# EdanToledo/Stoix

Hardware: AMD Instinct MI355X
Metric: env steps/sec (whole node), Anakin PPO on Brax Ant at 1/2/4/8 MI355X (higher is better)
Workload: dtype bf16; 1 GPU; model=ppo_mlp_256x2_tanh_normal, global_batch=4096, seq_len=128, parallelism=dp1, env=brax/ant, epochs=4, num_minibatches=16

## Files before the change

stoix_amd/ops/csrc/bind.cpp:

```cpp
#include <torch/extension.h>
#include <ATen/hip/HIPContext.h>

#include <cstdint>

extern "C" {
void launch_cartpole_step(float*, const long*, int*, float*, int*, float*,
                          int*, float*, float*, float*, float*, unsigned char*,
                          unsigned char*, int, int, uint64_t, unsigned int*,
                          unsigned int, int, void*);
void launch_ant_step(float*, const float*, int*, float*, int*, float*, int*,
                     float*, float*, float*, float*, unsigned char*,
                     unsigned char*, int, int, uint64_t, unsigned int*,
                     unsigned int, int, void*);
void launch_humanoid_step(float*, const float*, int*, float*, int*, float*,
                          int*, float*, float*, float*, float*,
                          unsigned char*, unsigned char*, int, int, uint64_t,
                          unsigned int*, unsigned int, int, void*);
void launch_ant_reset(float*, int, uint64_t, uint32_t, void*);
void launch_gae(const float*, const float*, const float*, const float*,
                const unsigned char*, float*, float*, int, int, float, void*);
void launch_lambda_returns(const float*, const float*, const float*, float*,
                           int, int, float, void*);
void launch_vtrace(const float*, const float*, const float*, const float*,
                   const float*, float*, float*, int, int, float, float,
// ... 30 lines not shown
                             float, float, float, uint64_t, uint64_t,
                             unsigned int*, unsigned int*, unsigned int,
                             void*);
void launch_linear_silu(const void*, const void*, const float*, void*,
                        void*, int, int, int, int, void*);
void launch_silu_fwd(const void*, void*, long, void*);
void launch_silu_bwd(const void*, const void*, void*, long, void*);
void launch_silu_heads_fwd(const void*, const void*, const void*, const void*,
                           const void*, void*, void*, void*, int, int, void*);
void launch_heads_bwd_silu(const void*, const void*, const void*, const void*,
                           const void*, void*, int, int, void*);
void launch_ppo_gather(const long*, int, const float*, int, int,
                       const float*, int,
                       const float*, const float*, const float*, const float*,
                       void*, float*, float*, float*, float*, float*,
                       const float*, const float*, void*);
void launch_ppo_head_loss(const void*, const void*, const float*,
                          const float*, const float*, const float*,
                          const float*, void*, void*, void*, float*, int,
                          int, float, float, float, float, float, float,
                          float, uint64_t, unsigned int*, unsigned int, int,
                          void*);
void launch_wgrad(const void*, const void*, float*, long, long, long, int,
                  int, int, int, int, int, void*);
void launch_slab_reduce(float*, void*, long, long, float*, long*, void*);
void launch_bump_add(unsigned int*, unsigned int, void*);
void launch_tr16_probe(const void*, float*, int, void*);
int launch_wgrad_pair(const void*, const void*, float*, long, long, long, int,
                      const void*, const void*, float*, long, long, long, int,
                      int, int, int, int, void*);
void launch_slab_reduce_pair(const float*, void*, long, long, float*, long*,
                             const float*, void*, long, long, float*, long*,
                             void*);
void launch_sumtree_update(float*, const long*, const float*, long, int, int,
                           void*);
void launch_sumtree_sample(const float*, const float*, long*, long, int, int,
                           int, void*);
void launch_policy_value_step_disc(const float*, const void*, const float*,
                                   const void*, const float*, const void*,
                                   const float*, const void*, const float*,
                                   const void*, const float*, const void*,
                                   const float*, float*, long*, float*,
                                   float*, const float*, const float*, int,
                                   int, int, int, int, uint64_t,
                                   unsigned int*, unsigned int, int, void*);
void launch_ppo_head_loss_disc(const void*, const void*, const long*,
                               const float*, const float*, const float*,
                               const float*, void*, void*, void*, float*,
                               int, int, float, float, float, void*);
void launch_ppo_gather_disc(const long*, int, const float*, int, int,
                            const long*, const float*, const float*,
                            const float*, const float*, void*, long*, float*,
                            float*, float*, float*, const float*,
                            const float*, void*);
void launch_rnn_scan(const float*, const void*, const float*,
                     const unsigned char*, const float*, const float*,
                     float*, float*, float*, int, int, int, int, void*);
void launch_rnn_scan_train_fwd(const float*, const void*, const float*,
                               const unsigned char*, const float*,
                               const float*, float*, float*, float*, float*,
                               float*, int, int, int, int, void*);
void launch_rnn_scan_bwd(const float*, const float*, const float*,
                         const float*, const float*, const float*,
                         const float*, const float*, const unsigned char*,
                         const void*, float*, float*, float*, float*, int,
                         int, int, int, void*);
// ... 420 lines not shown
  launch_rollout_step_ant(
      obs_io.data_ptr<float>(), env_state.data_ptr<float>(),
      step_count.data_ptr<int>(), ep_return.data_ptr<float>(),
      ep_length.data_ptr<int>(), last_ep_return.data_ptr<float>(),
      last_ep_length.data_ptr<int>(), W1a.data_ptr(), b1a.data_ptr<float>(),
      W2a.data_ptr(), b2a.data_ptr<float>(), Wha.data_ptr(),
      bha.data_ptr<float>(), W1c.data_ptr(), b1c.data_ptr<float>(),
      W2c.data_ptr(), b2c.data_ptr<float>(), Wvc.data_ptr(),
      bvc.data_ptr<float>(), buf_obs.data_ptr<float>(),
      buf_action.data_ptr<float>(), buf_logp.data_ptr<float>(),
      buf_value.data_ptr<float>(), buf_bootstrap.data_ptr<float>(),
      buf_reward.data_ptr<float>(), buf_discount.data_ptr<float>(),
      buf_steptype.data_ptr<unsigned char>(), B, OBS, ACT, HID,
      (int)max_episode_steps, (float)min_scale, (float)aff_scale,
      (float)aff_shift, (float)log_aff_scale, (uint64_t)policy_seed,
      (uint64_t)env_seed, (unsigned int*)policy_draw.data_ptr<int>(),
      (unsigned int*)env_draw.data_ptr<int>(), (unsigned int)draw_offset,
      cur_stream());
}

void linear_silu(torch::Tensor X, torch::Tensor W, torch::Tensor bias,
                 torch::Tensor Z, torch::Tensor H, int64_t do_silu) {
  CHK(X, torch::kBFloat16);
  CHK(W, torch::kBFloat16);
  CHK(bias, torch::kFloat32);
  int S = X.size(0), K = X.size(1), N = W.size(0);
  TORCH_CHECK(S % 128 == 0 && N % 128 == 0 && K % 32 == 0,
              "linear_silu tile constraints");
  void* h = H.numel() > 0 ? H.data_ptr() : nullptr;
  launch_linear_silu(X.data_ptr(), W.data_ptr(), bias.data_ptr<float>(),
                     Z.data_ptr(), h, S, K, N, (int)do_silu, cur_stream());
}

void silu_fwd(torch::Tensor z, torch::Tensor h) {
  CHK(z, torch::kBFloat16);
  TORCH_CHECK(z.numel() % 8 == 0, "silu_fwd needs numel % 8 == 0");
  launch_silu_fwd(z.data_ptr(), h.data_ptr(), z.numel(), cur_stream());
}

void silu_bwd(torch::Tensor dh, torch::Tensor z, torch::Tensor dz) {
  CHK(z, torch::kBFloat16);
  TORCH_CHECK(z.numel() % 8 == 0, "silu_bwd needs numel % 8 == 0");
  launch_silu_bwd(dh.data_ptr(), z.data_ptr(), dz.data_ptr(), z.numel(),
                  cur_stream());
}

int check_stacked_heads(const torch::Tensor& Z2, const torch::Tensor& other,
                        const torch::Tensor& Wh, const torch::Tensor& Wv,
                        const torch::Tensor& rows16, const torch::Tensor& rows1,
                        bool rows1_optional, int* hid) {
  CHK(Z2, torch::kBFloat16);
  CHK(other, torch::kBFloat16);
  CHK(rows16, torch::kBFloat16);
  CHK(rows1, torch::kBFloat16);
  TORCH_CHECK(Z2.dim() == 3 && Z2.size(0) == 2,
              "fused heads need stacked [2, S, HID] buffers");
  const int64_t S = Z2.size(1), HID = Z2.size(2);
  TORCH_CHECK(HID == 512 || HID == 256 || HID == 128,
              "fused heads support HID 128/256/512, got ", HID);
  TORCH_CHECK(S % 16 == 0, "fused heads need S % 16 == 0, got ", S);
  TORCH_CHECK(other.sizes() == Z2.sizes(),
              "fused heads: [2, S, HID] buffers differ in shape");
  check_fused_weight(Wh, "Wh", 16, HID);
  check_fused_weight(Wv.view({-1, 1}), "Wv", HID, 1);
  TORCH_CHECK(rows16.numel() == S * 16, "fused heads: expected [S, 16]");
  TORCH_CHECK(rows1.numel() == S || (rows1_optional && rows1.numel() == 0),
// ... 141 lines not shown
  wgrad_pair_slab_check(slab1, dW_off1, db_off1, n_valid1, K);
  return launch_wgrad_pair(
             dZ0.data_ptr(), X0.data_ptr(), slab0.data_ptr<float>(),
             (long)dW_off0, (long)db_off0, (long)slab0.size(1), (int)n_valid0,
             dZ1.data_ptr(), X1.data_ptr(), slab1.data_ptr<float>(),
             (long)dW_off1, (long)db_off1, (long)slab1.size(1), (int)n_valid1,
             (int)S, (int)N_STRIDE, (int)K, (int)variant, cur_stream()) != 0;
}

void slab_reduce_pair(torch::Tensor slab0, torch::Tensor grad0,
                      torch::Tensor sqnorm0, torch::Tensor step0,
                      torch::Tensor slab1, torch::Tensor grad1,
                      torch::Tensor sqnorm1, torch::Tensor step1) {
  CHK(slab0, torch::kFloat32);
  CHK(grad0, torch::kBFloat16);
  CHK(slab1, torch::kFloat32);
  CHK(grad1, torch::kBFloat16);
  TORCH_CHECK(slab0.dim() == 2 && slab0.size(0) == 64 && slab1.dim() == 2 &&
                  slab1.size(0) == 64, "slab_reduce_pair: slabs must be [64, n]");
  TORCH_CHECK(grad0.numel() <= slab0.size(1) && grad1.numel() <= slab1.size(1),
              "slab_reduce_pair: grad longer than a slab image");
  TORCH_CHECK((sqnorm0.numel() > 0) == (step0.numel() > 0) &&
                  (sqnorm1.numel() > 0) == (step1.numel() > 0),
              "slab_reduce_pair: sqnorm and step_t go together");
  float* sq0 = sqnorm0.numel() > 0 ? sqnorm0.data_ptr<float>() : nullptr;
  long* st0 = step0.numel() > 0 ? step0.data_ptr<long>() : nullptr;
  float* sq1 = sqnorm1.numel() > 0 ? sqnorm1.data_ptr<float>() : nullptr;
  long* st1 = step1.numel() > 0 ? step1.data_ptr<long>() : nullptr;
  launch_slab_reduce_pair(slab0.data_ptr<float>(), grad0.data_ptr(),
                          slab0.size(1), grad0.numel(), sq0, st0,
                          slab1.data_ptr<float>(), grad1.data_ptr(),
                          slab1.size(1), grad1.numel(), sq1, st1,
                          cur_stream());
}

void bump_add(torch::Tensor draw_buf, int64_t n) {
  launch_bump_add((unsigned int*)draw_buf.data_ptr<int>(), (unsigned int)n,
                  cur_stream());
}

void tr16_probe(torch::Tensor in, torch::Tensor out, int64_t base_mode) {
  CHK(in, torch::kBFloat16);
  launch_tr16_probe(in.data_ptr(), out.data_ptr<float>(), (int)base_mode,
                    cur_stream());
}

int check_c51_logits(const torch::Tensor& logits, const char* name,
                     int64_t B, int64_t A) {
  TORCH_CHECK(logits.is_cuda() && logits.is_contiguous(), name,
              " must be a contiguous GPU tensor");
  TORCH_CHECK(logits.scalar_type() == torch::kFloat32 ||
                  logits.scalar_type() == torch::kBFloat16,
              name, " must be fp32 or bf16");
  TORCH_CHECK(logits.dim() == 3 && logits.size(0) == B && logits.size(1) == A,
              name, " must be [", B, ", ", A, ", atoms]");
  TORCH_CHECK(A >= 1 && A <= 64, "c51 loss supports 1 <= A <= 64, got ", A);
  TORCH_CHECK(logits.size(2) >= 1 && logits.size(2) <= 1024,
              "c51 loss supports 1 <= atoms <= 1024, got ", logits.size(2));
  return logits.scalar_type() == torch::kBFloat16 ? 1 : 0;
}

void check_c51_vector(const torch::Tensor& t, const char* name,
                      torch::ScalarType ty, int64_t B) {
  TORCH_CHECK(t.is_cuda() && t.scalar_type() == ty && t.dim() == 1 &&
                  t.size(0) == B && t.stride(0) >= 0,
              name, " must be a GPU vector of ", B, " ", ty, " values");
// ... 389 lines not shown
        "fused clip + Adam, bf16 grads + bf16 param mirror");
  m.def("polyak", &polyak, "polyak target update");
  m.def("mfma_probe", &mfma_probe, "MFMA 16x16x32 bf16 layout probe");
  m.def("policy_value_step", &policy_value_step,
        "fused actor+critic fwd + tanh-normal sample (MFMA)");
  m.def("value_forward", &value_forward, "fused critic fwd (MFMA)");
  m.def("rollout_step_ant", &rollout_step_ant,
        "fused rollout step: policy + Ant physics + bootstrap, one launch");
  m.def("linear_silu", &linear_silu,
        "fused Linear(+bias)+SiLU forward, MFMA tiled");
  m.def("silu_fwd", &silu_fwd, "bf16 silu forward");
  m.def("silu_bwd", &silu_bwd, "bf16 silu backward");
  m.def("silu_heads_fwd", &silu_heads_fwd,
        "stacked silu forward fused with the actor/critic head GEMMs");
  m.def("heads_bwd_silu", &heads_bwd_silu,
        "head dgrads (K=16 / K=1) fused with the stacked silu backward");
  m.def("ppo_gather", &ppo_gather, "fused minibatch gather");
  m.def("ppo_head_loss", &ppo_head_loss,
        "fused PPO head fwd + losses + analytic head bwd");
  m.def("wgrad", &wgrad, "split-K MFMA weight grad + bias colsum -> slab",
        py::arg("dZ"), py::arg("X"), py::arg("slab"), py::arg("dW_off"),
        py::arg("db_off"), py::arg("n_valid"), py::arg("kpg") = 0,
        py::arg("ntb") = 0);
  m.def("slab_reduce", &slab_reduce,
        "sum wgrad slabs into flat bf16 grads (+ fused Adam prologue)");
  m.def("wgrad_pair", &wgrad_pair,
        "both nets' split-K wgrads in one pipelined launch -> slabs",
        py::arg("dZ0"), py::arg("X0"), py::arg("slab0"), py::arg("dW_off0"),
        py::arg("db_off0"), py::arg("n_valid0"), py::arg("dZ1"),
        py::arg("X1"), py::arg("slab1"), py::arg("dW_off1"),
        py::arg("db_off1"), py::arg("n_valid1"), py::arg("variant") = -1);
  m.def("slab_reduce_pair", &slab_reduce_pair,
        "both chains' slabs -> flat bf16 grads, slabs left un-zeroed");
  m.def("bump_add", &bump_add, "add N to a device RNG draw counter");
  m.def("tr16_probe", &tr16_probe, "ds_read_tr16_b64 semantics probe");
}
```

stoix_amd/ops/csrc/mlp.hip:

```cpp
#include "common.h"
#include "ant_core.h"
#include <hip/hip_bf16.h>
#include <stdexcept>
#include <string>
#include <type_traits>

typedef __bf16 bf16_t;
typedef __bf16 bf16x8 __attribute__((ext_vector_type(8)));
typedef __bf16 bf16x4 __attribute__((ext_vector_type(4)));
typedef float f32x4 __attribute__((ext_vector_type(4)));

#define MFMA_BF16_16x16x32 __builtin_amdgcn_mfma_f32_16x16x32_bf16

DEV_INLINE float bf2f(bf16_t x) { return (float)x; }
DEV_INLINE bf16_t f2bf(float x) { return (bf16_t)x; }

DEV_INLINE float silu_f(float x) {
  float s = 1.0f / (1.0f + __expf(-x));
  return x * s;
}
DEV_INLINE float silu_grad_f(float x) {
  float s = 1.0f / (1.0f + __expf(-x));
  return s * (1.0f + x * (1.0f - s));
}
// ... 587 lines not shown
    int n = n_blk + wn + nj * 16 + col_l;
    float bv = bias[n];
#pragma unroll
    for (int mi = 0; mi < 4; ++mi) {
#pragma unroll
      for (int r = 0; r < 4; ++r) {
        int m = m0 + wm + mi * 16 + g * 4 + r;
        float z = acc[mi][nj][r] + bv;
        Z[(long)m * N + n] = f2bf(z);
        if (SILU && H) H[(long)m * N + n] = f2bf(silu_f(z));
      }
    }
  }
}

extern "C" void launch_linear_silu(const void* X, const void* W,
                                   const float* bias, void* Z, void* H,
                                   int S, int K, int N, int do_silu,
                                   void* stream) {
  dim3 grid(S / LSF_BM, N / 128), block(256);
  if (do_silu) {
    hipLaunchKernelGGL(linear_silu_kernel<true>, grid, block, 0,
                       (hipStream_t)stream, (const bf16_t*)X,
                       (const bf16_t*)W, bias, (bf16_t*)Z, (bf16_t*)H, S, K,
                       N);
  } else {
    hipLaunchKernelGGL(linear_silu_kernel<false>, grid, block, 0,
                       (hipStream_t)stream, (const bf16_t*)X,
                       (const bf16_t*)W, bias, (bf16_t*)Z, (bf16_t*)H, S, K,
                       N);
  }
}


extern "C" __global__ void silu_fwd_kernel(const bf16_t* __restrict__ z,
                                           bf16_t* __restrict__ h, long n) {
  long i = ((long)blockIdx.x * blockDim.x + threadIdx.x) * 8;
  long stride = (long)gridDim.x * blockDim.x * 8;
  for (; i < n; i += stride) {
    bf16x8 zv = *reinterpret_cast<const bf16x8*>(z + i);
    bf16x8 hv;
#pragma unroll
    for (int j = 0; j < 8; ++j) hv[j] = f2bf(silu_f(bf2f(zv[j])));
    *reinterpret_cast<bf16x8*>(h + i) = hv;
  }
}

extern "C" __global__ void silu_bwd_kernel(const bf16_t* __restrict__ dh,
                                           const bf16_t* __restrict__ z,
                                           bf16_t* __restrict__ dz, long n) {
  long i = ((long)blockIdx.x * blockDim.x + threadIdx.x) * 8;
  long stride = (long)gridDim.x * blockDim.x * 8;
  for (; i < n; i += stride) {
    bf16x8 dv = *reinterpret_cast<const bf16x8*>(dh + i);
    bf16x8 zv = *reinterpret_cast<const bf16x8*>(z + i);
    bf16x8 o;
#pragma unroll
    for (int j = 0; j < 8; ++j)
      o[j] = f2bf(bf2f(dv[j]) * silu_grad_f(bf2f(zv[j])));
    *reinterpret_cast<bf16x8*>(dz + i) = o;
  }
}


DEV_INLINE void wave_lds_sync() {
  __builtin_amdgcn_fence(__ATOMIC_ACQ_REL, "wavefront");
// ... 768 lines not shown
```

stoix_amd/ops/csrc/optim.hip:

```cpp
#include "common.h"

extern "C" __global__ void grad_sqnorm_kernel(
    const float* __restrict__ grad, float* __restrict__ out, long n) {
  long tid = (long)blockIdx.x * blockDim.x + threadIdx.x;
  long stride = (long)gridDim.x * blockDim.x;
  float acc = 0.0f;
  long nvec = n / 4;
  const float4* g4 = reinterpret_cast<const float4*>(grad);
  for (long v = tid; v < nvec; v += stride) {
    float4 g = g4[v];
    acc += g.x * g.x + g.y * g.y + g.z * g.z + g.w * g.w;
  }
  for (long j = nvec * 4 + tid; j < n; j += stride) acc += grad[j] * grad[j];
#pragma unroll
  for (int off = 32; off > 0; off >>= 1) acc += __shfl_down(acc, off);
  __shared__ float warp_sums[16];
  int lane = threadIdx.x & 63;
  int wid = threadIdx.x >> 6;
  if (lane == 0) warp_sums[wid] = acc;
  __syncthreads();
  if (threadIdx.x == 0) {
    float s = 0.0f;
    int nw = (blockDim.x + 63) / 64;
    for (int w = 0; w < nw; ++w) s += warp_sums[w];
// ... 126 lines not shown
}

extern "C" void launch_fused_adam_bf16(float* param, const void* grad,
                                       float* exp_avg, float* exp_avg_sq,
                                       float* sqnorm, long* step_t,
                                       void* param_bf16, long n, float lr,
                                       float beta1, float beta2, float eps,
                                       float max_norm, float grad_scale,
                                       int do_prologue, long sqnorm_len,
                                       void* stream) {
  hipStream_t s = (hipStream_t)stream;
  if (do_prologue)
    hipLaunchKernelGGL(adam_prologue_kernel, dim3(1), dim3(1), 0, s, sqnorm,
                       step_t);
  int threads = 256;
  long want = (n / 8 + threads - 1) / threads;
  int blocks = (int)(want < 2048 ? (want > 0 ? want : 1) : 2048);
  int n_partials = 0;
  if (max_norm > 0.0f) {
    bool ordered = sqnorm_len >= 1 + (long)blocks;
    if (ordered) n_partials = blocks;
    hipLaunchKernelGGL(grad_sqnorm_bf16_kernel, dim3(blocks), dim3(threads),
                       0, s, (const opt_bf16*)grad, sqnorm,
                       ordered ? sqnorm + 1 : (float*)nullptr, n);
  }
  long want2 = (n + threads - 1) / threads;
  int blocks2 = (int)(want2 < 2048 ? (want2 > 0 ? want2 : 1) : 2048);
  hipLaunchKernelGGL(adam_update_bf16_kernel, dim3(blocks2), dim3(threads), 0,
                     s, param, (const opt_bf16*)grad, exp_avg, exp_avg_sq,
                     sqnorm, step_t, (opt_bf16*)param_bf16, n, lr, beta1,
                     beta2, eps, max_norm, grad_scale, n_partials);
}

extern "C" __global__ void polyak_kernel(const float* __restrict__ online,
                                         float* __restrict__ target,
                                         long n, float tau) {
  long i = (long)blockIdx.x * blockDim.x + threadIdx.x;
  long stride = (long)gridDim.x * blockDim.x;
  for (; i < n; i += stride)
    target[i] = tau * online[i] + (1.0f - tau) * target[i];
}

extern "C" void launch_fused_adam(float* param, const float* grad,
                                  float* exp_avg, float* exp_avg_sq,
                                  float* sqnorm, long* step_t, long n,
                                  float lr, float beta1, float beta2,
                                  float eps, float max_norm, void* stream) {
  hipStream_t s = (hipStream_t)stream;
  hipLaunchKernelGGL(adam_prologue_kernel, dim3(1), dim3(1), 0, s, sqnorm, step_t);
  int threads = 256;
  long want = (n / 4 + threads - 1) / threads;
  int blocks = (int)(want < 2048 ? (want > 0 ? want : 1) : 2048);
  if (max_norm > 0.0f) {
    hipLaunchKernelGGL(grad_sqnorm_kernel, dim3(blocks), dim3(threads), 0, s,
                       grad, sqnorm, n);
  }
  long want2 = (n + threads - 1) / threads;
  int blocks2 = (int)(want2 < 2048 ? (want2 > 0 ? want2 : 1) : 2048);
  hipLaunchKernelGGL(adam_update_kernel, dim3(blocks2), dim3(threads), 0, s,
                     param, grad, exp_avg, exp_avg_sq, sqnorm, step_t, n, lr,
                     beta1, beta2, eps, max_norm);
}

extern "C" void launch_polyak(const float* online, float* target, long n,
                              float tau, void* stream) {
  int threads = 256;
// ... 6 lines not shown
```

stoix_amd/ops/csrc/wgrad.hip:

```cpp
#include "common.h"
#include <cstdlib>
#include <hip/hip_bf16.h>

typedef __bf16 bf16_t;
typedef __bf16 bf16x8 __attribute__((ext_vector_type(8)));
typedef __bf16 bf16x4 __attribute__((ext_vector_type(4)));
typedef float f32x4 __attribute__((ext_vector_type(4)));

#define MFMA_BF16_16x16x32 __builtin_amdgcn_mfma_f32_16x16x32_bf16

#define WG_SLICES 64
#define SPAD 8

struct WgradLds {
  bf16_t dZt[4][4 * 16][32 + SPAD];
  bf16_t Xt[4][8 * 16][32 + SPAD];
};

template <int KPG, int NTB>
__launch_bounds__(256, 2) __global__ void wgrad_kernel(
    const bf16_t* __restrict__ dZ,
    const bf16_t* __restrict__ X,
    float* __restrict__ slab,
    long dW_off,
// ... 297 lines not shown
      d += __shfl_xor(d, 32);
      if (g == 0 && nb + col < N_VALID) out[db_off + nb + col] = d;
    }
  }
}

extern "C" __launch_bounds__(256) __global__ void slab_reduce_pair_kernel(
    const float* __restrict__ slab0, __bf16* __restrict__ grad0, long stride0,
    long n0, float* __restrict__ sqnorm0, long* __restrict__ step0,
    const float* __restrict__ slab1, __bf16* __restrict__ grad1, long stride1,
    long n1, float* __restrict__ sqnorm1, long* __restrict__ step1) {
  const bool second = blockIdx.y != 0;
  const float* __restrict__ slab = second ? slab1 : slab0;
  __bf16* __restrict__ grad16 = second ? grad1 : grad0;
  const long slab_stride = second ? stride1 : stride0;
  const long n = second ? n1 : n0;
  float* sqnorm = second ? sqnorm1 : sqnorm0;
  long* step_t = second ? step1 : step0;
  if (sqnorm && blockIdx.x == 0 && threadIdx.x == 0) {
    *sqnorm = 0.0f;
    *step_t += 1;
  }
  long i = (long)blockIdx.x * blockDim.x + threadIdx.x;
  long stride = (long)gridDim.x * blockDim.x;
  for (; i < n; i += stride) {
    float v[WG_SLICES];
#pragma unroll
    for (int z = 0; z < WG_SLICES; ++z) v[z] = slab[(long)z * slab_stride + i];
    float s = 0.0f;
#pragma unroll
    for (int z = 0; z < WG_SLICES; ++z) s += v[z];
    grad16[i] = (__bf16)s;
  }
}

extern "C" __global__ void tr16_probe_kernel(const bf16_t* __restrict__ in,
                                             float* __restrict__ out,
                                             int base_mode) {
  __shared__ bf16_t l[1024];
  int t = threadIdx.x;
  for (int i = t; i < 1024; i += 64) l[i] = in[i];
  __syncthreads();
  if (t >= 64) return;
  int off = 0;
  if (base_mode == 1) off = (t >> 4) * 64;
  else if (base_mode == 2) off = (t >> 4) * 128;
  bf16x4 v = __builtin_amdgcn_ds_read_tr16_b64_v4bf16(
      (__attribute__((address_space(3))) bf16x4*)&l[off]);
#pragma unroll
  for (int j = 0; j < 4; ++j) out[t * 4 + j] = (float)v[j];
}


extern "C" void launch_wgrad(const void* dZ, const void* X, float* slab,
                             long dW_off, long db_off, long slab_stride,
                             int S, int N_STRIDE, int K, int N_VALID,
                             int kpg_override, int ntb_override,
                             void* stream) {
  hipStream_t s = (hipStream_t)stream;
  int NT = (N_VALID + 15) / 16;
  int NTB = (NT % 4 == 0) ? 4 : 1;
  int KPG = 1;
  if (ntb_override > 0) NTB = ntb_override;
  if (kpg_override > 0) {
    KPG = kpg_override;
  } else if (NT <= 1) {
// ... 128 lines not shown
```

stoix_amd/systems/ppo/fused.py:

```python
from __future__ import annotations

import math
from typing import Dict, List, Optional, Tuple

import torch
import torch.nn as nn
import torch.nn.functional as F

from stoix_amd.networks.heads import NormalAffineTanhDistributionHead, ScalarCriticHead
from stoix_amd.networks.torso import MLPTorso

Tensor = torch.Tensor


def _mlp_linears(torso: nn.Module) -> Optional[List[nn.Linear]]:
    if not isinstance(torso, MLPTorso):
        return None
    lins = [m for m in torso.net if isinstance(m, nn.Linear)]
    acts = [m for m in torso.net if isinstance(m, nn.SiLU)]
    if len(lins) != 2 or len(acts) != 2 or len(list(torso.net)) != 4:
        return None
    return lins


class _Chain:

    def __init__(
        self,
        specs: List[Tuple[str, Tuple[int, ...]]],
        device,
        lr: float,
        flat16: Optional[Tensor] = None,
        grad16: Optional[Tensor] = None,
    ):
        self.lr = lr
        sizes = [int(torch.prod(torch.tensor(s)).item()) for _, s in specs]
        total = sum(sizes)
        self.flat = torch.zeros(total, dtype=torch.float32, device=device)
        self.flat16 = (
            flat16 if flat16 is not None
            else torch.zeros(total, dtype=torch.bfloat16, device=device)
        )
        self.grad16 = (
            grad16 if grad16 is not None
            else torch.zeros(total, dtype=torch.bfloat16, device=device)
        )
        self.m = torch.zeros(total, dtype=torch.float32, device=device)
        self.v = torch.zeros(total, dtype=torch.float32, device=device)
        self.sqnorm = torch.zeros(1 + 2048, dtype=torch.float32, device=device)
        self.step_t = torch.zeros(1, dtype=torch.int64, device=device)
        self.views: Dict[str, Tensor] = {}
        self.views16: Dict[str, Tensor] = {}
        self.gviews16: Dict[str, Tensor] = {}
        self.offsets: Dict[str, int] = {}
        off = 0
        for (name, shape), n in zip(specs, sizes):
            self.views[name] = self.flat[off : off + n].view(*shape)
            self.views16[name] = self.flat16[off : off + n].view(*shape)
            self.gviews16[name] = self.grad16[off : off + n].view(*shape)
            self.offsets[name] = off
            off += n
        self.numel = total
        self.slab = torch.zeros(64, total, dtype=torch.float32, device=device)

    def sync_mirror(self) -> None:
        self.flat16.copy_(self.flat)


class FusedPPOEngine:

    @staticmethod
    def try_build(learner) -> Optional["FusedPPOEngine"]:
        if learner.device.type != "cuda":
            return None
        if type(learner).policy_loss is not _base_policy_loss_func(learner):
            return None
        actor, critic = learner.actor, learner.critic
        if actor.input_layer is not None or critic.input_layer is not None:
            return None
        a_lins = _mlp_linears(actor.torso)
        c_lins = _mlp_linears(critic.torso)
        if a_lins is None or c_lins is None:
# ... 149 lines not shown
                ws.val = z(S, dtype=torch.float32)
                ws.adv = z(S, dtype=torch.float32)
                ws.tgt = z(S, dtype=torch.float32)

        self.ws = [_Ws(), _Ws()]
        self.Xmb = self.ws[0].Xmb
        self.act_mb = self.ws[0].act
        self.logp_mb = self.ws[0].logp
        self.val_mb = self.ws[0].val
        self.adv_mb = self.ws[0].adv
        self.tgt_mb = self.ws[0].tgt
        self.gather_stream = torch.cuda.Stream(dev)
        self.ev_ready = [torch.cuda.Event(), torch.cuda.Event()]
        self.ev_consumed = [torch.cuda.Event(), torch.cuda.Event()]
        self.Z1, self.H1 = z(2, S, H), z(2, S, H)
        self.Z2, self.H2 = z(2, S, H), z(2, S, H)
        self.dH2 = z(2, S, H)
        self.dZ2 = z(2, S, H)
        self.dH1 = z(2, S, H)
        self.dZ1 = z(2, S, H)
        self.heads = z(S, 16)
        self.vpred = z(S, 1)
        self.dhead = z(S, 16)
        self.dv = z(S, 1)
        self.dv16 = z(S, 16)

        import os as _os

        self.use_bmm = _os.environ.get("STOIX_FUSED_BMM", "1") != "0"
        _heads = _os.environ.get("STOIX_FUSED_HEADS", "1")
        self.fused_heads = _heads != "0"
        self.fused_vpred = _heads == "2"
        self.fused_wgrad = _os.environ.get("STOIX_FUSED_WGRAD", "1") != "0"
        self.no_vpred = z(0)
        self.prefetch = _os.environ.get("STOIX_FUSED_PREFETCH", "0") == "1"

        import torch.distributed as dist

        self.world = dist.get_world_size() if dist.is_initialized() else 1

        self.norm = bool(getattr(learner, "normalize_obs", False))
        if self.norm:
            st = learner.obs_stats
            self.nmean = st.mean
            self.nvar = (st.std ** 2).clone()
            self.gmean = st.mean.clone()
            self.gvar = self.nvar.clone()

        learner.env._hb["obs"].copy_(learner.cur_obs)


    def _adopt_params(self, a_lins, c_lins, head, critic_head) -> None:
        ac, cc = self.actor_chain, self.critic_chain
        ACT, H = self.ACT, self.H
        OBS = self.OBS
        with torch.no_grad():
            ac.views["W1"].zero_()
            cc.views["W1"].zero_()
            ac.views["W1"][:, :OBS].copy_(a_lins[0].weight)
            ac.views["b1"].copy_(a_lins[0].bias)
            ac.views["W2"].copy_(a_lins[1].weight)
            ac.views["b2"].copy_(a_lins[1].bias)
            ac.views["Wh"].zero_()
            ac.views["bh"].zero_()
            if self.discrete:
                ac.views["Wh"][0:ACT].copy_(head.linear.weight)
                ac.views["bh"][0:ACT].copy_(head.linear.bias)
            else:
                ac.views["Wh"][0:ACT].copy_(head.loc.weight)
                ac.views["Wh"][8 : 8 + ACT].copy_(head.scale.weight)
                ac.views["bh"][0:ACT].copy_(head.loc.bias)
                ac.views["bh"][8 : 8 + ACT].copy_(head.scale.bias)
            cc.views["W1"][:, :OBS].copy_(c_lins[0].weight)
            cc.views["b1"].copy_(c_lins[0].bias)
            cc.views["W2"].copy_(c_lins[1].weight)
            cc.views["b2"].copy_(c_lins[1].bias)
            cc.views["Wv"].copy_(critic_head.linear.weight.view(-1))
            cc.views["bv"].copy_(critic_head.linear.bias)
        a_lins[0].weight.data = ac.views["W1"][:, :OBS]
        a_lins[0].bias.data = ac.views["b1"]
        a_lins[1].weight.data = ac.views["W2"]
        a_lins[1].bias.data = ac.views["b2"]
# ... 125 lines not shown
            else L.buf_action.view(TB, self.ACT)
        )
        flat_logp = L.buf_log_prob.view(TB)
        flat_value = L.buf_value.view(TB)
        flat_adv = L.buf_adv.view(TB)
        flat_tgt = L.buf_targets.view(TB)
        ac, cc = self.actor_chain, self.critic_chain
        a16, c16 = ac.views16, cc.views16
        ag, cg = ac.gviews16, cc.gviews16

        import torch.distributed as dist

        gather_fn = ext.ppo_gather_disc if self.discrete else ext.ppo_gather
        gmean = self.gmean if self.norm else self.empty
        gvar = self.gvar if self.norm else self.empty

        def gather_into(mb: int, w) -> None:
            idx = L.perm_buf[mb * S : (mb + 1) * S]
            gather_fn(
                idx, flat_obs, flat_action, flat_logp, flat_value, flat_adv,
                flat_tgt, w.Xmb, w.act, w.logp, w.val, w.adv, w.tgt,
                gmean, gvar,
            )

        gs = self.gather_stream
        cur = torch.cuda.current_stream(self.device)
        prefetch = self.prefetch
        if prefetch:
            gs.wait_stream(cur)
            with torch.cuda.stream(gs):
                gather_into(0, self.ws[0])
                self.ev_ready[0].record(gs)

        for mb in range(n_mb):
            p = mb & 1 if prefetch else 0
            w = self.ws[p]
            if prefetch:
                cur.wait_event(self.ev_ready[p])
            else:
                gather_into(mb, w)
            ext.linear_silu(w.Xmb, a16["W1"], ac.views["b1"], self.Z1[0], self.H1[0], 1)
            ext.linear_silu(w.Xmb, c16["W1"], cc.views["b1"], self.Z1[1], self.H1[1], 1)
            torch.addmm(a16["b2"], self.H1[0], a16["W2"].t(), out=self.Z2[0])
            torch.addmm(c16["b2"], self.H1[1], c16["W2"].t(), out=self.Z2[1])
            if self.fused_heads:
                ext.silu_heads_fwd(
                    self.Z2, a16["Wh"], a16["bh"], c16["Wv"], c16["bv"],
                    self.H2, self.heads,
                    self.vpred if self.fused_vpred else self.no_vpred)
                if not self.fused_vpred:
                    torch.addmm(c16["bv"], self.H2[1],
                                c16["Wv"].view(self.H, 1), out=self.vpred)
            else:
                ext.silu_fwd(self.Z2, self.H2)
                torch.addmm(a16["bh"], self.H2[0], a16["Wh"].t(),
                            out=self.heads)
                torch.addmm(c16["bv"], self.H2[1], c16["Wv"].view(self.H, 1),
                            out=self.vpred)
            last = mb == n_mb - 1
            if last:
                self.metrics.zero_()
            if self.discrete:
                ext.ppo_head_loss_disc(
                    self.heads, self.vpred.view(-1), w.act, w.logp,
                    w.val, w.adv, w.tgt, self.dhead, self.dv,
                    self.dv16, self.metrics if last else self.metrics_none,
                    self.ACT, self.clip_eps, self.ent_coef, self.vf_coef,
                )
            else:
                ext.ppo_head_loss(
                    self.heads, self.vpred.view(-1), w.act, w.logp,
                    w.val, w.adv, w.tgt, self.dhead, self.dv,
                    self.dv16, self.metrics if last else self.metrics_none,
                    self.clip_eps, self.ent_coef,
                    self.vf_coef, self.min_scale, self.aff_scale, self.aff_shift,
# ... 11 lines not shown
                ext.wgrad(self.dhead, self.H2[0], ac.slab, ao["Wh"], ao["bh"], 16)
                ext.wgrad(self.dv16, self.H2[1], cc.slab, co["Wv"], co["bv"], 1)
            if self.fused_heads:
                ext.heads_bwd_silu(self.dhead, self.dv, a16["Wh"], c16["Wv"],
                                   self.Z2, self.dZ2)
            else:
                ext.silu_bwd(self.dH2, self.Z2, self.dZ2)
            if pair:
                ext.wgrad_pair(self.dZ2[0], self.H1[0], ac.slab, ao["W2"], ao["b2"], self.H,
                               self.dZ2[1], self.H1[1], cc.slab, co["W2"], co["b2"], self.H)
            else:
                ext.wgrad(self.dZ2[0], self.H1[0], ac.slab, ao["W2"], ao["b2"], self.H)
                ext.wgrad(self.dZ2[1], self.H1[1], cc.slab, co["W2"], co["b2"], self.H)
            if self.use_bmm:
                torch.bmm(self.dZ2, self.W2pair, out=self.dH1)
            else:
                torch.mm(self.dZ2[0], a16["W2"], out=self.dH1[0])
                torch.mm(self.dZ2[1], c16["W2"], out=self.dH1[1])
            ext.silu_bwd(self.dH1, self.Z1, self.dZ1)
            if pair:
                ext.wgrad_pair(self.dZ1[0], w.Xmb, ac.slab, ao["W1"], ao["b1"], self.H,
                               self.dZ1[1], w.Xmb, cc.slab, co["W1"], co["b1"], self.H)
            else:
                ext.wgrad(self.dZ1[0], w.Xmb, ac.slab, ao["W1"], ao["b1"], self.H)
                ext.wgrad(self.dZ1[1], w.Xmb, cc.slab, co["W1"], co["b1"], self.H)
            if prefetch:
                self.ev_consumed[p].record(cur)
                if mb + 1 < n_mb:
                    q = (mb + 1) & 1
                    gs.wait_event(self.ev_consumed[q])
                    with torch.cuda.stream(gs):
                        gather_into(mb + 1, self.ws[q])
                        self.ev_ready[q].record(gs)
            if pair:
                ext.slab_reduce_pair(ac.slab, ac.grad16, ac.sqnorm, ac.step_t,
                                     cc.slab, cc.grad16, cc.sqnorm, cc.step_t)
            else:
                ext.slab_reduce(ac.slab, ac.grad16, ac.sqnorm, ac.step_t)
                ext.slab_reduce(cc.slab, cc.grad16, cc.sqnorm, cc.step_t)
            if self.world > 1:
                dist.all_reduce(self.biggrad16)
            gscale = 1.0 / float(self.world)
            ext.fused_adam_bf16(
                ac.flat, ac.grad16, ac.m, ac.v, ac.sqnorm, ac.step_t,
                ac.flat16, ac.lr, 0.9, 0.999, 1e-5, self.max_grad_norm,
                gscale, 0,
            )
            ext.fused_adam_bf16(
                cc.flat, cc.grad16, cc.m, cc.v, cc.sqnorm, cc.step_t,
                cc.flat16, cc.lr, 0.9, 0.999, 1e-5, self.max_grad_norm,
                gscale, 0,
            )
        if prefetch:
            cur.wait_stream(gs)
        ext.bump_add(self.draw_ent, n_mb)
        return {k: v for k, v in self.metric_views.items()}


def _base_policy_loss_func(learner):
    from stoix_amd.systems.ppo import ff_ppo

    return ff_ppo.PPOLearner.policy_loss
```

Baseline: 25.07 million env_steps/s.

## Fuse actor/critic layer-1 forward, slab reduce with grad norm, and paired Adam

Adds a paired Linear+SiLU kernel that computes both actor and critic first layers over the shared minibatch input in one launch, storing through LDS for row-contiguous writes. Adds a slab reduction kernel that also computes each chain's squared gradient norm using a last-block-done counter, and a single Adam kernel covering both chains. The goal is fewer kernel launches and fewer separate norm passes per minibatch in the PPO update loop. The cost is extra complexity and atomic-counter state, and the tail path applies only for single-device runs with clipping enabled.

```diff
diff --git a/stoix_amd/ops/csrc/bind.cpp b/stoix_amd/ops/csrc/bind.cpp
--- a/stoix_amd/ops/csrc/bind.cpp
+++ b/stoix_amd/ops/csrc/bind.cpp
@@ -86,6 +86,17 @@
 void launch_slab_reduce_pair(const float*, void*, long, long, float*, long*,
                              const float*, void*, long, long, float*, long*,
                              void*);
+int launch_linear_silu_pair(const void*, const void*, const float*, void*,
+                            void*, const void*, const float*, void*, void*,
+                            int, int, int, void*);
+void launch_slab_reduce_norm_pair(const float*, void*, long, long, float*,
+                                  long*, unsigned int*, const float*, void*,
+                                  long, long, float*, long*, unsigned int*,
+                                  void*);
+void launch_adam_pair(float*, const void*, float*, float*, const float*,
+                      const long*, void*, long, float, float*, const void*,
+                      float*, float*, const float*, const long*, void*, long,
+                      float, float, float, float, float, float, void*);
 void launch_sumtree_update(float*, const long*, const float*, long, int, int,
                            void*);
 void launch_sumtree_sample(const float*, const float*, long*, long, int, int,
@@ -572,6 +583,41 @@
                      Z.data_ptr(), h, S, K, N, (int)do_silu, cur_stream());
 }
 
+bool linear_silu_pair(torch::Tensor X, torch::Tensor W_a, torch::Tensor b_a,
+                      torch::Tensor Z_a, torch::Tensor H_a, torch::Tensor W_c,
+                      torch::Tensor b_c, torch::Tensor Z_c,
+                      torch::Tensor H_c) {
+  CHK(X, torch::kBFloat16);
+  CHK(W_a, torch::kBFloat16);
+  CHK(W_c, torch::kBFloat16);
+  CHK(b_a, torch::kFloat32);
+  CHK(b_c, torch::kFloat32);
+  CHK(Z_a, torch::kBFloat16);
+  CHK(H_a, torch::kBFloat16);
+  CHK(Z_c, torch::kBFloat16);
+  CHK(H_c, torch::kBFloat16);
+  TORCH_CHECK(X.dim() == 2 && W_a.dim() == 2 && W_c.dim() == 2,
+              "linear_silu_pair: X and W must be 2-D");
+  const int64_t S = X.size(0), K = X.size(1), N = W_a.size(0);
+  TORCH_CHECK(W_a.size(1) == K && W_c.size(0) == N && W_c.size(1) == K,
+              "linear_silu_pair: the two nets' weight shapes differ");
+  TORCH_CHECK(b_a.numel() == N && b_c.numel() == N,
+              "linear_silu_pair: bias length");
+  TORCH_CHECK(Z_a.numel() == S * N && H_a.numel() == S * N &&
+                  Z_c.numel() == S * N && H_c.numel() == S * N,
+              "linear_silu_pair: outputs must hold S * N elements");
+  TORCH_CHECK(K > 0 && K % 32 == 0,
+              "linear_silu_pair: K must be a multiple of 32");
+  for (const torch::Tensor* t : {&X, &W_a, &W_c, &Z_a, &H_a, &Z_c, &H_c})
+    TORCH_CHECK(reinterpret_cast<uintptr_t>(t->data_ptr()) % 16 == 0,
+                "linear_silu_pair: operands must be 16-byte aligned");
+  return launch_linear_silu_pair(
+             X.data_ptr(), W_a.data_ptr(), b_a.data_ptr<float>(),
+             Z_a.data_ptr(), H_a.data_ptr(), W_c.data_ptr(),
+             b_c.data_ptr<float>(), Z_c.data_ptr(), H_c.data_ptr(), (int)S,
+             (int)K, (int)N, cur_stream()) == 0;
+}
+
 void silu_fwd(torch::Tensor z, torch::Tensor h) {
   CHK(z, torch::kBFloat16);
   TORCH_CHECK(z.numel() % 8 == 0, "silu_fwd needs numel % 8 == 0");
@@ -779,6 +825,94 @@
                           slab1.data_ptr<float>(), grad1.data_ptr(),
                           slab1.size(1), grad1.numel(), sq1, st1,
                           cur_stream());
+}
+
+constexpr int64_t kTailMaxN = 2048LL * 256 * 8;
+
+void slab_reduce_norm_pair(torch::Tensor slab0, torch::Tensor grad0,
+                           torch::Tensor sqnorm0, torch::Tensor step0,
+                           torch::Tensor counter0, torch::Tensor slab1,
+                           torch::Tensor grad1, torch::Tensor sqnorm1,
+                           torch::Tensor step1, torch::Tensor counter1) {
+  CHK(slab0, torch::kFloat32);
+  CHK(grad0, torch::kBFloat16);
+  CHK(sqnorm0, torch::kFloat32);
+  CHK(step0, torch::kInt64);
+  CHK(counter0, torch::kInt32);
+  CHK(slab1, torch::kFloat32);
+  CHK(grad1, torch::kBFloat16);
+  CHK(sqnorm1, torch::kFloat32);
+  CHK(step1, torch::kInt64);
+  CHK(counter1, torch::kInt32);
+  TORCH_CHECK(slab0.dim() == 2 && slab0.size(0) == 64 && slab1.dim() == 2 &&
+                  slab1.size(0) == 64,
+              "slab_reduce_norm_pair: slabs must be [64, n]");
+  const int64_t n0 = grad0.numel(), n1 = grad1.numel();
+  TORCH_CHECK(n0 >= 1 && n1 >= 1 && n0 <= slab0.size(1) && n1 <= slab1.size(1),
+              "slab_reduce_norm_pair: grad empty or longer than a slab image");
+  TORCH_CHECK(n0 <= kTailMaxN && n1 <= kTailMaxN,
+              "slab_reduce_norm_pair: chain too long for the ordered norm");
+  TORCH_CHECK(sqnorm0.numel() >= 1 + (n0 + 511) / 512 &&
+                  sqnorm1.numel() >= 1 + (n1 + 511) / 512,
+              "slab_reduce_norm_pair: sqnorm needs 1 + ceil(n / 512) floats");
+  TORCH_CHECK(step0.numel() == 1 && step1.numel() == 1 &&
+                  counter0.numel() == 1 && counter1.numel() == 1,
+              "slab_reduce_norm_pair: step_t and counter hold one element");
+  launch_slab_reduce_norm_pair(
+      slab0.data_ptr<float>(), grad0.data_ptr(), slab0.size(1), n0,
+      sqnorm0.data_ptr<float>(), step0.data_ptr<long>(),
+      (unsigned int*)counter0.data_ptr<int>(), slab1.data_ptr<float>(),
+      grad1.data_ptr(), slab1.size(1), n1, sqnorm1.data_ptr<float>(),
+      step1.data_ptr<long>(), (unsigned int*)counter1.data_ptr<int>(),
+      cur_stream());
+}
+
+void adam_pair(torch::Tensor param0, torch::Tensor grad0, torch::Tensor m0,
+               torch::Tensor v0, torch::Tensor sqnorm0, torch::Tensor step0,
+               torch::Tensor param_bf16_0, double lr0, torch::Tensor param1,
+               torch::Tensor grad1, torch::Tensor m1, torch::Tensor v1,
+               torch::Tensor sqnorm1, torch::Tensor step1,
+               torch::Tensor param_bf16_1, double lr1, double beta1,
+               double beta2, double eps, double max_norm, double grad_scale) {
+  CHK(param0, torch::kFloat32);
+  CHK(grad0, torch::kBFloat16);
+  CHK(m0, torch::kFloat32);
+  CHK(v0, torch::kFloat32);
+  CHK(sqnorm0, torch::kFloat32);
+  CHK(step0, torch::kInt64);
+  CHK(param1, torch::kFloat32);
+  CHK(grad1, torch::kBFloat16);
+  CHK(m1, torch::kFloat32);
+  CHK(v1, torch::kFloat32);
+  CHK(sqnorm1, torch::kFloat32);
+  CHK(step1, torch::kInt64);
+  const int64_t n0 = param0.numel(), n1 = param1.numel();
+  TORCH_CHECK(grad0.numel() == n0 && m0.numel() == n0 && v0.numel() == n0 &&
+                  grad1.numel() == n1 && m1.numel() == n1 && v1.numel() == n1,
+              "adam_pair: param, grad and moments must have one length");
+  TORCH_CHECK(sqnorm0.numel() >= 1 && sqnorm1.numel() >= 1 &&
+                  step0.numel() == 1 && step1.numel() == 1,
+              "adam_pair: sqnorm and step_t must not be empty");
+  void* pbf0 = nullptr;
+  void* pbf1 = nullptr;
+  if (param_bf16_0.numel() > 0) {
+    CHK(param_bf16_0, torch::kBFloat16);
+    TORCH_CHECK(param_bf16_0.numel() == n0, "adam_pair: bf16 mirror length");
+    pbf0 = param_bf16_0.data_ptr();
+  }
+  if (param_bf16_1.numel() > 0) {
+    CHK(param_bf16_1, torch::kBFloat16);
+    TORCH_CHECK(param_bf16_1.numel() == n1, "adam_pair: bf16 mirror length");
+    pbf1 = param_bf16_1.data_ptr();
+  }
+  launch_adam_pair(param0.data_ptr<float>(), grad0.data_ptr(),
+                   m0.data_ptr<float>(), v0.data_ptr<float>(),
+                   sqnorm0.data_ptr<float>(), step0.data_ptr<long>(), pbf0, n0,
+                   (float)lr0, param1.data_ptr<float>(), grad1.data_ptr(),
+                   m1.data_ptr<float>(), v1.data_ptr<float>(),
+                   sqnorm1.data_ptr<float>(), step1.data_ptr<long>(), pbf1, n1,
+                   (float)lr1, (float)beta1, (float)beta2, (float)eps,
+                   (float)max_norm, (float)grad_scale, cur_stream());
 }
 
 void bump_add(torch::Tensor draw_buf, int64_t n) {
@@ -1234,6 +1368,14 @@
         py::arg("db_off1"), py::arg("n_valid1"), py::arg("variant") = -1);
   m.def("slab_reduce_pair", &slab_reduce_pair,
         "both chains' slabs -> flat bf16 grads, slabs left un-zeroed");
+  m.def("linear_silu_pair", &linear_silu_pair,
+        "both nets' Linear(+bias)+SiLU forward over one X, row-contiguous "
+        "stores; false = shape not taken, nothing launched");
+  m.def("slab_reduce_norm_pair", &slab_reduce_norm_pair,
+        "slab_reduce_pair + each chain's ordered squared grad norm");
+  m.def("adam_pair", &adam_pair,
+        "both chains' clip + Adam + bf16 mirror in one launch");
+  m.attr("TAIL_MAX_N") = kTailMaxN;
   m.def("bump_add", &bump_add, "add N to a device RNG draw counter");
   m.def("tr16_probe", &tr16_probe, "ds_read_tr16_b64 semantics probe");
 }
diff --git a/stoix_amd/ops/csrc/mlp.hip b/stoix_amd/ops/csrc/mlp.hip
--- a/stoix_amd/ops/csrc/mlp.hip
+++ b/stoix_amd/ops/csrc/mlp.hip
@@ -643,6 +643,150 @@
   }
 }
 
+struct LinSiluNet {
+  const bf16_t* W;
+  const float* bias;
+  bf16_t* Z;
+  bf16_t* H;
+};
+
+#define LSP_TILE_BYTES (64 * 128)
+
+DEV_INLINE void wave_lds_sync();
+
+template <bool ACT>
+DEV_INLINE void lsp_store_tile(const f32x4 (&acc)[4][4], unsigned char* tile,
+                               bf16_t* __restrict__ out, int N, int lane) {
+  const int i = lane & 15, g = lane >> 4;
+#pragma unroll
+  for (int mi = 0; mi < 4; ++mi) {
+#pragma unroll
+    for (int nj = 0; nj < 4; ++nj) {
+      bf16x4 v;
+#pragma unroll
+      for (int r = 0; r < 4; ++r) {
+        const float z = acc[mi][nj][r];
+        v[r] = f2bf(ACT ? silu_f(z) : z);
+      }
+      const int chunk = (nj * 2 + (g >> 1)) ^ (i & 7);
+      const int half = (g & 1) ^ (i >> 3);
+      *reinterpret_cast<bf16x4*>(tile + (mi * 16 + i) * 128 + chunk * 16 +
+                                 half * 8) = v;
+    }
+  }
+  wave_lds_sync();
+  const int r8 = lane >> 3, c = lane & 7;
+#pragma unroll
+  for (int it = 0; it < 8; ++it) {
+    const int R = it * 8 + r8;
+    const bf16x8 t = *reinterpret_cast<const bf16x8*>(tile + R * 128 +
+                                                      ((c ^ r8) * 16));
+    const bf16x8 v = (it & 1)
+                         ? __builtin_shufflevector(t, t, 4, 5, 6, 7, 0, 1, 2, 3)
+                         : t;
+    *reinterpret_cast<bf16x8*>(out + (long)R * N + c * 8) = v;
+  }
+  wave_lds_sync();
+}
+
+__launch_bounds__(256, 2) __global__ void linear_silu_pair_kernel(
+    const bf16_t* __restrict__ X,
+    LinSiluNet net0, LinSiluNet net1, int S, int K, int N) {
+  constexpr int A_BYTES = 2 * LSF_BM * (LSF_BK + LSF_APAD) * 2;
+  constexpr int T_BYTES = 4 * LSP_TILE_BYTES;
+  __shared__ alignas(16) unsigned char smem[A_BYTES > T_BYTES ? A_BYTES
+                                                               : T_BYTES];
+  typedef bf16_t ATile[LSF_BM][LSF_BK + LSF_APAD];
+  ATile* A = reinterpret_cast<ATile*>(smem);
+  const LinSiluNet net = blockIdx.z ? net1 : net0;
+  const bf16_t* __restrict__ W = net.W;
+  const int lane = threadIdx.x & 63;
+  const int wid = threadIdx.x >> 6;
+  const int m0 = blockIdx.x * LSF_BM;
+  const int n_blk = blockIdx.y * 128;
+  const int wm = (wid >> 1) * 64;
+  const int wn = (wid & 1) * 64;
+  const int KS = K / LSF_BK;
+
+  f32x4 acc[4][4];
+#pragma unroll
+  for (int i = 0; i < 4; ++i)
+#pragma unroll
+    for (int j = 0; j < 4; ++j) acc[i][j] = {0.f, 0.f, 0.f, 0.f};
+
+  auto stage = [&](int ks, int pp) {
+#pragma unroll
+    for (int q = 0; q < 2; ++q) {
+      int flat = q * 256 + threadIdx.x;
+      int row = flat >> 2;
+      int kh = (flat & 3) * 8;
+      *reinterpret_cast<bf16x8*>(&A[pp][row][kh]) =
+          *reinterpret_cast<const bf16x8*>(X + (long)(m0 + row) * K +
+                                           ks * LSF_BK + kh);
+    }
+  };
+
+  stage(0, 0);
+  const int xrow_base = wm + (lane & 15);
+  const int ak0 = (lane >> 4) * 8;
+  for (int ks = 0; ks < KS; ++ks) {
+    __syncthreads();
+    if (ks + 1 < KS) stage(ks + 1, (ks + 1) & 1);
+    bf16x8 w[4];
+#pragma unroll
+    for (int nj = 0; nj < 4; ++nj) {
+      int n = n_blk + wn + nj * 16 + (lane & 15);
+      w[nj] = *reinterpret_cast<const bf16x8*>(W + (long)n * K +
+                                               ks * LSF_BK + ak0);
+    }
+#pragma unroll
+    for (int mi = 0; mi < 4; ++mi) {
+      const bf16x8 x = *reinterpret_cast<const bf16x8*>(
+          &A[ks & 1][xrow_base + mi * 16][ak0]);
+#pragma unroll
+      for (int nj = 0; nj < 4; ++nj) {
+        acc[mi][nj] = MFMA_BF16_16x16x32(w[nj], x, acc[mi][nj], 0, 0, 0);
+      }
+    }
+  }
+
+  const int g = lane >> 4;
+#pragma unroll
+  for (int nj = 0; nj < 4; ++nj) {
+    const float* bp = net.bias + n_blk + wn + nj * 16 + g * 4;
+    const float b0 = bp[0], b1 = bp[1], b2 = bp[2], b3 = bp[3];
+#pragma unroll
+    for (int mi = 0; mi < 4; ++mi) {
+      acc[mi][nj][0] += b0;
+      acc[mi][nj][1] += b1;
+      acc[mi][nj][2] += b2;
+      acc[mi][nj][3] += b3;
+    }
+  }
+
+  __syncthreads();
+  unsigned char* tile = smem + wid * LSP_TILE_BYTES;
+  const long o = (long)(m0 + wm) * N + n_blk + wn;
+  lsp_store_tile<false>(acc, tile, net.Z + o, N, lane);
+  lsp_store_tile<true>(acc, tile, net.H + o, N, lane);
+}
+
+extern "C" int launch_linear_silu_pair(const void* X, const void* W0,
+                                       const float* b0, void* Z0, void* H0,
+                                       const void* W1, const float* b1,
+                                       void* Z1, void* H1, int S, int K, int N,
+                                       void* stream) {
+  if (S <= 0 || S % LSF_BM != 0 || N <= 0 || N % 128 != 0 || K <= 0 ||
+      K % LSF_BK != 0)
+    return 1;
+  LinSiluNet n0{(const bf16_t*)W0, b0, (bf16_t*)Z0, (bf16_t*)H0};
+  LinSiluNet n1{(const bf16_t*)W1, b1, (bf16_t*)Z1, (bf16_t*)H1};
+  dim3 grid(S / LSF_BM, N / 128, 2), block(256);
+  hipLaunchKernelGGL(linear_silu_pair_kernel, grid, block, 0,
+                     (hipStream_t)stream, (const bf16_t*)X, n0, n1, S, K, N);
+  return 0;
+}
+
 
 extern "C" __global__ void silu_fwd_kernel(const bf16_t* __restrict__ z,
                                            bf16_t* __restrict__ h, long n) {
diff --git a/stoix_amd/ops/csrc/optim.hip b/stoix_amd/ops/csrc/optim.hip
--- a/stoix_amd/ops/csrc/optim.hip
+++ b/stoix_amd/ops/csrc/optim.hip
@@ -182,6 +182,71 @@
                      beta2, eps, max_norm, grad_scale, n_partials);
 }
 
+struct AdamChain {
+  float* param;
+  const opt_bf16* grad;
+  float* exp_avg;
+  float* exp_avg_sq;
+  const float* sqnorm;
+  const long* step_t;
+  opt_bf16* param_bf16;
+  long n;
+  float lr;
+};
+
+extern "C" __global__ void adam_pair_kernel(AdamChain c0, AdamChain c1,
+                                            float beta1, float beta2,
+                                            float eps, float max_norm,
+                                            float grad_scale) {
+  const AdamChain c = blockIdx.y ? c1 : c0;
+  float* __restrict__ param = c.param;
+  const opt_bf16* __restrict__ grad = c.grad;
+  float* __restrict__ exp_avg = c.exp_avg;
+  float* __restrict__ exp_avg_sq = c.exp_avg_sq;
+  opt_bf16* __restrict__ param_bf16 = c.param_bf16;
+  const long n = c.n;
+  const float lr = c.lr;
+  long i = (long)blockIdx.x * blockDim.x + threadIdx.x;
+  long stride = (long)gridDim.x * blockDim.x;
+  float clip = grad_scale;
+  if (max_norm > 0.0f) {
+    float sq = *c.sqnorm;
+    float norm = sqrtf(sq) * grad_scale;
+    if (norm > max_norm) clip = grad_scale * max_norm / (norm + 1e-6f);
+  }
+  long t = *c.step_t;
+  float bc1 = 1.0f - powf(beta1, (float)t);
+  float bc2 = 1.0f - powf(beta2, (float)t);
+  for (; i < n; i += stride) {
+    float g = (float)grad[i] * clip;
+    float m = exp_avg[i] = beta1 * exp_avg[i] + (1.0f - beta1) * g;
+    float v = exp_avg_sq[i] = beta2 * exp_avg_sq[i] + (1.0f - beta2) * g * g;
+    float p = param[i] - lr * (m / bc1) / (sqrtf(v / bc2) + eps);
+    param[i] = p;
+    if (param_bf16) param_bf16[i] = (opt_bf16)p;
+  }
+}
+
+extern "C" void launch_adam_pair(
+    float* param0, const void* grad0, float* exp_avg0, float* exp_avg_sq0,
+    const float* sqnorm0, const long* step0, void* param_bf16_0, long n0,
+    float lr0, float* param1, const void* grad1, float* exp_avg1,
+    float* exp_avg_sq1, const float* sqnorm1, const long* step1,
+    void* param_bf16_1, long n1, float lr1, float beta1, float beta2,
+    float eps, float max_norm, float grad_scale, void* stream) {
+  AdamChain c0{param0, (const opt_bf16*)grad0, exp_avg0, exp_avg_sq0, sqnorm0,
+               step0, (opt_bf16*)param_bf16_0, n0, lr0};
+  AdamChain c1{param1, (const opt_bf16*)grad1, exp_avg1, exp_avg_sq1, sqnorm1,
+               step1, (opt_bf16*)param_bf16_1, n1, lr1};
+  int threads = 256;
+  long nmax = n0 > n1 ? n0 : n1;
+  long want = (nmax + threads - 1) / threads;
+  int blocks = (int)(want < 2048 ? (want > 0 ? want : 1) : 2048);
+  hipLaunchKernelGGL(adam_pair_kernel, dim3(blocks, 2), dim3(threads), 0,
+                     (hipStream_t)stream, c0, c1, beta1, beta2, eps, max_norm,
+                     grad_scale);
+}
+
 extern "C" __global__ void polyak_kernel(const float* __restrict__ online,
                                          float* __restrict__ target,
                                          long n, float tau) {
diff --git a/stoix_amd/ops/csrc/wgrad.hip b/stoix_amd/ops/csrc/wgrad.hip
--- a/stoix_amd/ops/csrc/wgrad.hip
+++ b/stoix_amd/ops/csrc/wgrad.hip
@@ -353,6 +353,107 @@
     for (int z = 0; z < WG_SLICES; ++z) s += v[z];
     grad16[i] = (__bf16)s;
   }
+}
+
+struct TailChain {
+  const float* slab;
+  __bf16* grad16;
+  long slab_stride, n;
+  float* sqnorm;
+  long* step_t;
+  unsigned int* counter;
+};
+
+__device__ __forceinline__ float slab_sum(const float* __restrict__ slab,
+                                          long slab_stride, long i) {
+  float v[WG_SLICES];
+#pragma unroll
+  for (int z = 0; z < WG_SLICES; ++z) v[z] = slab[(long)z * slab_stride + i];
+  float s = 0.0f;
+#pragma unroll
+  for (int z = 0; z < WG_SLICES; ++z) s += v[z];
+  return s;
+}
+
+extern "C" __launch_bounds__(512) __global__
+    void slab_reduce_norm_pair_kernel(TailChain c0, TailChain c1) {
+  const TailChain c = blockIdx.y ? c1 : c0;
+  const long n = c.n;
+  const int nblk = (int)((n + 511) / 512);
+  if ((int)blockIdx.x >= nblk) return;
+  if (blockIdx.x == 0 && threadIdx.x == 0) *c.step_t += 1;
+  __shared__ float x[512];
+  __shared__ int is_last;
+  const long i = (long)blockIdx.x * 512 + threadIdx.x;
+  float xv = 0.0f;
+  if (i < n) {
+    const __bf16 q = (__bf16)slab_sum(c.slab, c.slab_stride, i);
+    c.grad16[i] = q;
+    xv = (float)q;
+  }
+  x[threadIdx.x] = xv;
+  __syncthreads();
+  const long nvec = n / 8;
+  if (threadIdx.x < 64) {
+    float acc = 0.0f;
+    if ((long)blockIdx.x * 64 + threadIdx.x < nvec) {
+#pragma unroll
+      for (int j = 0; j < 8; ++j) {
+        float v = x[threadIdx.x * 8 + j];
+        acc += v * v;
+      }
+    }
+    if (blockIdx.x == 0 && (long)threadIdx.x < n - nvec * 8) {
+      float v = (float)(__bf16)slab_sum(c.slab, c.slab_stride,
+                                        nvec * 8 + threadIdx.x);
+      acc += v * v;
+    }
+#pragma unroll
+    for (int off = 32; off > 0; off >>= 1) acc += __shfl_down(acc, off);
+    if (threadIdx.x == 0) {
+      __hip_atomic_store(c.sqnorm + 1 + blockIdx.x, acc, __ATOMIC_RELAXED,
+                         __HIP_MEMORY_SCOPE_AGENT);
+      asm volatile("s_waitcnt vmcnt(0)" ::: "memory");
+      is_last = __hip_atomic_fetch_add(c.counter, 1u, __ATOMIC_RELAXED,
+                                       __HIP_MEMORY_SCOPE_AGENT) ==
+                (unsigned int)(nblk - 1);
+    }
+  }
+  __syncthreads();
+  if (!is_last || threadIdx.x >= 64) return;
+  const long nb = nvec > 256 ? (nvec + 255) / 256 : 1;
+  float acc = 0.0f;
+  for (long p = threadIdx.x; p < nb; p += 64) {
+    float s = 0.0f;
+#pragma unroll
+    for (int w = 0; w < 4; ++w) {
+      const long b = 4 * p + w;
+      s += b < nblk ? __hip_atomic_load(c.sqnorm + 1 + b, __ATOMIC_RELAXED,
+                                        __HIP_MEMORY_SCOPE_AGENT)
+                    : 0.0f;
+    }
+    acc += s;
+  }
+#pragma unroll
+  for (int off = 32; off > 0; off >>= 1) acc += __shfl_down(acc, off);
+  if (threadIdx.x == 0) {
+    c.sqnorm[0] = acc;
+    __hip_atomic_store(c.counter, 0u, __ATOMIC_RELAXED,
+                       __HIP_MEMORY_SCOPE_AGENT);
+  }
+}
+
+extern "C" void launch_slab_reduce_norm_pair(
+    const float* slab0, void* grad0, long stride0, long n0, float* sqnorm0,
+    long* step0, unsigned int* counter0, const float* slab1, void* grad1,
+    long stride1, long n1, float* sqnorm1, long* step1,
+    unsigned int* counter1, void* stream) {
+  TailChain c0{slab0, (__bf16*)grad0, stride0, n0, sqnorm0, step0, counter0};
+  TailChain c1{slab1, (__bf16*)grad1, stride1, n1, sqnorm1, step1, counter1};
+  long nmax = n0 > n1 ? n0 : n1;
+  int blocks = (int)((nmax + 511) / 512);
+  hipLaunchKernelGGL(slab_reduce_norm_pair_kernel, dim3(blocks, 2), dim3(512),
+                     0, (hipStream_t)stream, c0, c1);
 }
 
 extern "C" __global__ void tr16_probe_kernel(const bf16_t* __restrict__ in,
diff --git a/stoix_amd/systems/ppo/fused.py b/stoix_amd/systems/ppo/fused.py
--- a/stoix_amd/systems/ppo/fused.py
+++ b/stoix_amd/systems/ppo/fused.py
@@ -47,7 +47,10 @@
         )
         self.m = torch.zeros(total, dtype=torch.float32, device=device)
         self.v = torch.zeros(total, dtype=torch.float32, device=device)
-        self.sqnorm = torch.zeros(1 + 2048, dtype=torch.float32, device=device)
+        self.sqnorm = torch.zeros(
+            1 + max(2048, (total + 511) // 512), dtype=torch.float32, device=device
+        )
+        self.tail_counter = torch.zeros(1, dtype=torch.int32, device=device)
         self.step_t = torch.zeros(1, dtype=torch.int64, device=device)
         self.views: Dict[str, Tensor] = {}
         self.views16: Dict[str, Tensor] = {}
@@ -263,6 +266,8 @@
         self.fused_heads = _heads != "0"
         self.fused_vpred = _heads == "2"
         self.fused_wgrad = _os.environ.get("STOIX_FUSED_WGRAD", "1") != "0"
+        self.fused_l1 = _os.environ.get("STOIX_FUSED_L1", "1") != "0"
+        self.fused_tail = _os.environ.get("STOIX_FUSED_TAIL", "1") != "0"
         self.no_vpred = z(0)
         self.prefetch = _os.environ.get("STOIX_FUSED_PREFETCH", "0") == "1"
 
@@ -279,6 +284,26 @@
             self.gvar = self.nvar.clone()
 
         learner.env._hb["obs"].copy_(learner.cur_obs)
+
+    def _tail_eligible(self) -> bool:
+        cap = int(self.ext.TAIL_MAX_N)
+        return (
+            self.fused_tail and self.fused_wgrad and self.world == 1
+            and self.max_grad_norm > 0.0
+            and self.actor_chain.numel <= cap and self.critic_chain.numel <= cap
+        )
+
+    def layer1_forward(self, Xmb: Tensor) -> None:
+        ext = self.ext
+        ac, cc = self.actor_chain, self.critic_chain
+        a16, c16 = ac.views16, cc.views16
+        if self.fused_l1 and ext.linear_silu_pair(
+            Xmb, a16["W1"], ac.views["b1"], self.Z1[0], self.H1[0],
+            c16["W1"], cc.views["b1"], self.Z1[1], self.H1[1],
+        ):
+            return
+        ext.linear_silu(Xmb, a16["W1"], ac.views["b1"], self.Z1[0], self.H1[0], 1)
+        ext.linear_silu(Xmb, c16["W1"], cc.views["b1"], self.Z1[1], self.H1[1], 1)
 
 
     def _adopt_params(self, a_lins, c_lins, head, critic_head) -> None:
@@ -470,6 +495,7 @@
                 gather_into(0, self.ws[0])
                 self.ev_ready[0].record(gs)
 
+        tail = self._tail_eligible()
         for mb in range(n_mb):
             p = mb & 1 if prefetch else 0
             w = self.ws[p]
@@ -477,8 +503,7 @@
                 cur.wait_event(self.ev_ready[p])
             else:
                 gather_into(mb, w)
-            ext.linear_silu(w.Xmb, a16["W1"], ac.views["b1"], self.Z1[0], self.H1[0], 1)
-            ext.linear_silu(w.Xmb, c16["W1"], cc.views["b1"], self.Z1[1], self.H1[1], 1)
+            self.layer1_forward(w.Xmb)
             torch.addmm(a16["b2"], self.H1[0], a16["W2"].t(), out=self.Z2[0])
             torch.addmm(c16["b2"], self.H1[1], c16["W2"].t(), out=self.Z2[1])
             if self.fused_heads:
@@ -556,6 +581,18 @@
                     with torch.cuda.stream(gs):
                         gather_into(mb + 1, self.ws[q])
                         self.ev_ready[q].record(gs)
+            if tail:
+                ext.slab_reduce_norm_pair(
+                    ac.slab, ac.grad16, ac.sqnorm, ac.step_t, ac.tail_counter,
+                    cc.slab, cc.grad16, cc.sqnorm, cc.step_t, cc.tail_counter)
+                ext.adam_pair(
+                    ac.flat, ac.grad16, ac.m, ac.v, ac.sqnorm, ac.step_t,
+                    ac.flat16, ac.lr,
+                    cc.flat, cc.grad16, cc.m, cc.v, cc.sqnorm, cc.step_t,
+                    cc.flat16, cc.lr,
+                    0.9, 0.999, 1e-5, self.max_grad_norm, 1.0,
+                )
+                continue
             if pair:
                 ext.slab_reduce_pair(ac.slab, ac.grad16, ac.sqnorm, ac.step_t,
                                      cc.slab, cc.grad16, cc.sqnorm, cc.step_t)
```

Measured after the change: 27.46 million env_steps/s, median of 6. 9.5% higher.
